# xmed-lab/MOC

Measured on AMD Instinct MI355X. Metric: meta-steps/sec (train), slides/sec (eval) on 16-shot NSCLC synthetic bags, higher is better.
Workload: dtype f32; 1 GPU; NSCLC 2-way 16-shot train loop: 32 slides/epoch x 15000 patches x 512, topj 400, topk 10, row mask on; bag_storage=fp32, arithmetic=fp32 accumulate (MFMA), parallelism=single GPU, one Adam step per slide

## Files before the change

### moc_amd/csrc/moc_meta.hip

```cpp
#include <cstdlib>
#include <cstring>
#include <new>
#include "moc_meta_internal.h"
#include <type_traits>
#include "moc_p2p.h"

int moc_check_batch(const moc_batch_t* B, const char* who);
int moc_launch_topk_mean(const float* keys, int64_t key_stride, const float* vals, int64_t val_stride,
                         const int64_t* seg_off, const int32_t* seg_len, int seg0, int n_seg, int C, int K,
                         int smallest, float* pooled, int32_t* idx_out, int32_t* cnt_out, hipStream_t s);

using namespace moc_meta_internal;

namespace {

struct AdamCoef {
    float wd, one_minus_b1, beta2, one_minus_b2, eps;
    float neg_step_size;
    float bc2_sqrt;
    float grad_scale;
};

__device__ __forceinline__ void adam_update(float& p, float& m, float& v, float g, const AdamCoef& k) {
    g = moc_fadd(g, moc_fmul(k.wd, p));
// ... 634 lines not shown
        for (int sw = 0; sw < 2; ++sw) {
            const int d = dl + sw * dcols;
            if (d < D) {
                float g0 = 0.f, g1 = 0.f;
                for (int p = 0; p < P; ++p) {
                    const float xv = xs[(size_t)p * D + d];
                    g0 = fmaf(dhs[p * H + ha], xv, g0);
                    if (JN > 1) g1 = fmaf(dhs[p * H + ha + 1], xv, g1);
                }
                gr[sw][0] = g0; gr[sw][1] = g1;
            }
        }
    }
    float gt = 0.f;
    int tail = -1;
    if (wg == 0) {
        if (t < 4 * H) {
            const int i = t >> 6, h = t & 63;
            for (int p = 0; p < P; ++p) gt = fmaf(dz[p * 4 + i], H1s[p * H + h], gt);
            tail = H + t;
        } else if (t < 4 * H + 4) {
            const int i = t - 4 * H;
            for (int p = 0; p < P; ++p) gt += dz[p * 4 + i];
            tail = H + 4 * H + i;
        } else if (t >= 320 && t < 320 + H) {
            const int h = t - 320;
            for (int p = 0; p < P; ++p) gt += dhs[p * H + h];
            tail = h;
        }
    }
    if (!a.apply_adam) {
        if (own)
            for (int sw = 0; sw < 2; ++sw) {
                const int d = dl + sw * dcols;
                if (d < D) { g.g_W1[(ha + 0) * D + d] = gr[sw][0]; if (JN > 1) g.g_W1[(ha + 1) * D + d] = gr[sw][1]; }
            }
        if (tail >= H + 4 * H) a.g_b2[tail - 5 * H] = gt;
        else if (tail >= H) a.g_W2[tail - H] = gt;
        else if (tail >= 0) a.g_b1[tail] = gt;
        return;
    }
    if (g.x.world > 1) {
        __shared__ int p2p_ok;
        const int64_t nW1 = (int64_t)H * D;
        if (own)
#pragma unroll
            for (int sw = 0; sw < 2; ++sw) {
                const int d = dl + sw * dcols;
                if (d < D) { p2p_push(g.x, (int64_t)(ha + 0) * D + d, gr[sw][0]); if (JN > 1) p2p_push(g.x, (int64_t)(ha + 1) * D + d, gr[sw][1]); }
            }
        if (tail >= 0) p2p_push(g.x, nW1 + tail, gt);
        if (!p2p_signal_wait(g.x, wg, &p2p_ok)) return;
        if (own)
#pragma unroll
            for (int sw = 0; sw < 2; ++sw) {
                const int d = dl + sw * dcols;
                if (d < D) {
                    gr[sw][0] = p2p_sum(g.x, (int64_t)(ha + 0) * D + d, gr[sw][0]);
                    if (JN > 1) gr[sw][1] = p2p_sum(g.x, (int64_t)(ha + 1) * D + d, gr[sw][1]);
                }
            }
        if (tail >= 0) gt = p2p_sum(g.x, nW1 + tail, gt);
    }
    const float gs = ak.grad_scale;
    if (own) {
#pragma unroll
        for (int sw = 0; sw < 2; ++sw) {
            const int d = dl + sw * dcols;
            if (d < D) {
#pragma unroll
                for (int j = 0; j < 2; ++j) {
                    if (j >= JN) continue;
                    const int e = (ha + j) * D + d;
                    adam_update(pw[j][sw], pm[j][sw], pv[j][sw], gr[sw][j] * gs, ak);
                    g.W1[e] = pw[j][sw]; g.m_W1[e] = pm[j][sw]; g.v_W1[e] = pv[j][sw];
                    w1_image_store(g.img_dt, g.W1img, D, ha + j, d, pw[j][sw]);
                }
            }
        }
    }
    if (tail >= 0) {
        adam_update(pW, pM, pV, gt * gs, ak);
        if (tail >= H + 4 * H) { const int i = tail - 5 * H; a.b2[i] = pW; a.m_b2[i] = pM; a.v_b2[i] = pV; }
        else if (tail >= H) { const int i = tail - H; g.W2out[i] = pW; a.m_W2[i] = pM; a.v_W2[i] = pV; }
        else { a.b1[tail] = pW; a.m_b1[tail] = pM; a.v_b1[tail] = pV; }
    }
    MOC_STAMP(18);
}

struct TileStepArgs {
    const unsigned long long* tkey;
    const uint32_t* trho;
    int64_t slot0;
    int cap, ntile_bound, C, K, D, slide0;
    int n_runs, slide_stride;
    const int32_t* n_sel;
    const int64_t* labels;
    int PS_CAP, xdt;
    int tail_inside;
    int S_host;
    float *W1, *m_W1, *v_W1;
    const float* W2;
    float *b1, *m_b1, *v_b1, *b2, *m_b2, *v_b2, *m_W2, *v_W2;
    int64_t base;
    AdamCoef adam;
    const AdamCoef* adam_tab;
    const int32_t* adam_ctr;
    int adam_pos, apply_adam;
    uint32_t use_bits;
    int img_dt;
    const int64_t* trid;
    const float4* tlam;
    const float4* tsc;
    const float* H1;
    const unsigned char* X;
    float* pooled_out;
    int32_t* topk_idx_out;
    int32_t* topk_cnt_out;
    float* loss;
    int32_t* pred;
    int32_t* n_pair;
    unsigned char* W1img;
    float* W2out;
    float *g_W1, *g_b1, *g_W2, *g_b2;
    const float* mixed_in;
    const float* cand;
    const float* gates;
    const int64_t* sel_row;
    int64_t stride;
    int64_t par_stride, w2_stride, w2out_stride, img_stride;
    const int64_t* row_off;
    int prefetch_next;
    int sink_off;
};
struct TileStepArgsRuns {
    TileStepArgs s;
    int64_t base_r[MOC_MAX_RUNS], slot0_r[MOC_MAX_RUNS];
    int32_t cap_r[MOC_MAX_RUNS], ntb_r[MOC_MAX_RUNS];
};
static_assert(sizeof(TileStepArgsRuns) <= 1024, "a kernel-argument segment over 1 KiB takes a slow launch path (profiles/NOTES.md)");
constexpr int MOC_HP_RUNS = 8;
struct TileStepArgsRunsHp {
    TileStepArgs s;
    int64_t base_r[MOC_HP_RUNS], slot0_r[MOC_HP_RUNS];
    int32_t cap_r[MOC_HP_RUNS], ntb_r[MOC_HP_RUNS];
    AdamCoef adam_r[MOC_HP_RUNS];
};
static_assert(sizeof(TileStepArgsRunsHp) <= 1024, "a kernel-argument segment over 1 KiB takes a slow launch path (profiles/NOTES.md)");
static_assert(offsetof(TileStepArgsRunsHp, adam_r) % sizeof(AdamCoef) == 0, "a run's coefficients: one aligned 32-byte scalar load");
__host__ __device__ __forceinline__ const TileStepArgs& tile_common(const TileStepArgs& x) { return x; }
__host__ __device__ __forceinline__ const TileStepArgs& tile_common(const TileStepArgsRuns& x) { return x.s; }
__host__ __device__ __forceinline__ const TileStepArgs& tile_common(const TileStepArgsRunsHp& x) { return x.s; }

template <int VQ, typename ArgsT>
__global__ __launch_bounds__(256, 4) void pool_w1_step_tiles_kernel(ArgsT args) {
    extern __shared__ __attribute__((aligned(16))) unsigned char smem[];
    constexpr bool RUNS = !std::is_same<ArgsT, TileStepArgs>::value;
    constexpr bool RUN_HP = std::is_same<ArgsT, TileStepArgsRunsHp>::value;
    const TileStepArgs& a = tile_common(args);
    static_assert(offsetof(TileStepArgs, n_sel) + 8 <= 64, "the first loads' arguments must share the first cache line");
    int b = a.slide0;
    int64_t base = 0, slot0 = a.slot0, po = 0, w2o = 0, w2outo = 0, imgo = 0;
    int cap = a.cap, ntile_bound = a.ntile_bound;
    constexpr bool runs = RUNS;
    if constexpr (RUNS) {
        const int run = blockIdx.z;
        b += run * a.slide_stride;
        slot0 = kernarg_at<int64_t>(offsetof(ArgsT, slot0_r) + 8 * (size_t)run);
        cap = kernarg_at<int32_t>(offsetof(ArgsT, cap_r) + 4 * (size_t)run);
        ntile_bound = kernarg_at<int32_t>(offsetof(ArgsT, ntb_r) + 4 * (size_t)run);
    }
    const int C = a.C, K = a.K, D = a.D;
    const int t = threadIdx.x, lane = t & 63, wave = __builtin_amdgcn_readfirstlane(t >> 6);
    const int cb = blockIdx.x, h = blockIdx.y;
    const bool tail_wg = !a.tail_inside && cb == (D >> 8);
    const bool tail_role = a.tail_inside ? cb == 0 : tail_wg;
    const bool wg0 = cb == 0 && h == 0;
    constexpr int CL = 64;
    MOC_STAMP(10);
    MOC_STAMP_MIN(33);
    MOC_STAMP_MAX(34);
    unsigned long long key[VQ];
    uint32_t rho[VQ / 4];
#define MOC_TILE_KEYS(c)                                                                                              \
    {                                                                                                                 \
        const int64_t s_c_ = slot0 + (int64_t)(c) * cap * TILE_R;                                                     \
        const int nrec_b_ = ntile_bound * TILE_R;                                                                     \
        _Pragma("unroll") for (int q = 0; q < VQ; ++q) {                                                              \
            const int j = q * 64 + lane;                                                                              \
            key[q] = a.tkey[s_c_ + (j < nrec_b_ ? j : nrec_b_ - 1)];                                                  \
        }                                                                                                             \
        _Pragma("unroll") for (int rq = 0; rq < VQ / 4; ++rq) {                                                       \
            const int x = rq * 64 + lane;                                                                             \
            rho[rq] = a.trho[slot0 / TILE_R + (int64_t)(c) * cap + (x < ntile_bound ? x : ntile_bound - 1)];          \
        }                                                                                                             \
    }
    if (wave < C) MOC_TILE_KEYS(wave)
    __builtin_amdgcn_sched_barrier(0);
    moc_kernarg_touch<sizeof(ArgsT)>();
    const int PS_CAP = a.PS_CAP;
    base = a.base;
    if constexpr (RUNS) {
        const int run = blockIdx.z;
        base = kernarg_at<int64_t>(offsetof(ArgsT, base_r) + 8 * (size_t)run);
        po = (int64_t)run * a.par_stride; w2o = (int64_t)run * a.w2_stride; w2outo = (int64_t)run * a.w2out_stride;
        imgo = (int64_t)run * a.img_stride;
    }
    const int d = cb * 256 + t;
    float pw = 0.f, pm = 0.f, pv = 0.f;
    float pT = 0.f, pTm = 0.f, pTv = 0.f;
    int tail = -1;
    if (tail_role) {
        if (t < 4) tail = H + t * H + h;
        else if (t == 64) tail = h;
        else if (h == 0 && t >= 128 && t < 132) tail = H + 4 * H + (t - 128);
    }
    float w2v = 0.f;
    if (t < 4) w2v = a.W2[w2o + t * H + h];
    if (a.apply_adam) {
        if (!tail_wg) {
            const int64_t e = po + h * D + d;
            pw = a.W1[e]; pm = a.m_W1[e]; pv = a.v_W1[e];
        }
        if (tail >= H + 4 * H) { const int64_t i = po + tail - 5 * H; pT = a.b2[i]; pTm = a.m_b2[i]; pTv = a.v_b2[i]; }
        else if (tail >= H) { const int64_t i = po + tail - H; pTm = a.m_W2[i]; pTv = a.v_W2[i]; }
        else if (tail >= 0) { pT = a.b1[po + tail]; pTm = a.m_b1[po + tail]; pTv = a.v_b1[po + tail]; }
    }
    MOC_STAMP(19);
    if (wave >= C && a.prefetch_next) {
        const int64_t nb = a.row_off[b + 1];
        const int S2 = a.n_sel[b + 1];
        const int esz_p = a.xdt == MOC_F32 ? 4 : 2;
        const int lpr = D * esz_p / 128;
        const int iw = 4 - C;
        const int gx = (D >> 8) + (a.tail_inside ? 0 : 1);
        const int g0 = ((h * gx + cb) * iw + (wave - C)) * 64 + lane, G = gx * H * iw * 64;
        typedef const __attribute__((address_space(1))) void* gptr_t;
        typedef __attribute__((address_space(3))) void* lptr_t;
        float* sinkw = reinterpret_cast<float*>(smem + a.sink_off) + (wave - C) * 64;
        for (int L = g0; L < S2 * lpr; L += G) {
            const int r = L / lpr;
            const unsigned char* pl = a.X + a.sel_row[nb + r] * (int64_t)D * esz_p + (int64_t)(L - r * lpr) * 128;
            __builtin_amdgcn_global_load_lds((gptr_t)pl, (lptr_t)sinkw, 4, 0, 0);
        }
        const int ncol = 2 * C + 2, lpc = (S2 + 31) >> 5;
        for (int L = g0; L < ncol * lpc; L += G) {
            const int c = L / lpc;
            const float* pl = a.cand + (int64_t)c * a.stride + nb + (int64_t)(L - c * lpc) * 32;
            __builtin_amdgcn_global_load_lds((gptr_t)pl, (lptr_t)sinkw, 4, 0, 0);
        }
    }
    AdamCoef ak = a.adam;
    if (a.adam_tab) ak = a.adam_tab[a.adam_ctr[0] + a.adam_pos];
    if constexpr (RUN_HP) ak = kernarg_at<AdamCoef>(offsetof(ArgsT, adam_r) + sizeof(AdamCoef) * (size_t)blockIdx.z);
    const int S = (!RUNS && a.S_host >= 0) ? a.S_host : a.n_sel[b];
    const int y = (int)a.labels[b];
    const int k = K < S ? K : S;
    float4* plam = reinterpret_cast<float4*>(smem);
    float4* psc = plam + (size_t)C * K;
    float* xs = reinterpret_cast<float*>(psc + (size_t)C * K);
    float* dhs = xs + (size_t)C * K * 256;
    float* dz = dhs + (((size_t)C * K + 3) & ~(size_t)3);
    unsigned long long* list = reinterpret_cast<unsigned long long*>(dz + (size_t)C * K * 4);
    unsigned long long* t0s = list + (size_t)C * PS_CAP;
    int64_t* prid = reinterpret_cast<int64_t*>(t0s + C);
    int* lsrc = reinterpret_cast<int*>(prid + (size_t)C * K);
    float* topv = reinterpret_cast<float*>(lsrc + (size_t)C * CL);
    float* pooled_s = topv + (size_t)C * 16;
    float* dpool = pooled_s + C;
    int* ncand = reinterpret_cast<int*>(dpool + C);
    int* flagc = ncand + C;
    int* topk_s = flagc + C;
    float* h1s = reinterpret_cast<float*>(topk_s + C * K);
    float* w2s = h1s + (size_t)C * K;
    if (t < 4) { w2s[t] = w2v; if (tail >= H) pT = w2v; }
    const int ntile = (S + 15) >> 4;
    for (int c = wave; c < C; c += 4) {
        const int64_t s_c = slot0 + (int64_t)c * cap * TILE_R;
        if (c != wave) MOC_TILE_KEYS(c)
        if (lane == 0) ncand[c] = 0;
        uint32_t hi[VQ];
        uint32_t m = 0u;
        const int nrec = ntile * TILE_R;
#pragma unroll
        for (int q = 0; q < VQ; ++q) {
            hi[q] = q * 64 + lane < nrec ? (uint32_t)(key[q] >> 32) : 0u;
            m = hi[q] > m ? hi[q] : m;
        }
        MOC_STAMP(20);
        {
            const uint32_t o1 = (uint32_t)__builtin_amdgcn_update_dpp(0, (int)m, 0xB1, 0xf, 0xf, false);
            m = o1 > m ? o1 : m;
            const uint32_t o2 = (uint32_t)__builtin_amdgcn_update_dpp(0, (int)m, 0x4E, 0xf, 0xf, false);
            m = o2 > m ? o2 : m;
        }
        const uint32_t gm = (uint32_t)__shfl((int)m, (lane & 15) * 4, 64);
        int grank = 0;
#define MOC_ROR(n) grank += (uint32_t)__builtin_amdgcn_update_dpp(0, (int)gm, 0x120 + n, 0xf, 0xf, false) > gm ? 1 : 0;
        MOC_ROR(1) MOC_ROR(2) MOC_ROR(3) MOC_ROR(4) MOC_ROR(5) MOC_ROR(6) MOC_ROR(7) MOC_ROR(8)
        MOC_ROR(9) MOC_ROR(10) MOC_ROR(11) MOC_ROR(12) MOC_ROR(13) MOC_ROR(14) MOC_ROR(15)
#undef MOC_ROR
        const unsigned long long hit = __ballot(lane < 16 && grank == k - 1 && gm != 0u);
        uint32_t T0 = 0u;
        if (hit != 0ull) T0 = (uint32_t)__builtin_amdgcn_readlane((int)gm, __ffsll((long long)hit) - 1);
        const uint32_t T1 = T0 > 1u ? T0 : 1u;
        int cnt = 0;
#pragma unroll
        for (int q = 0; q < VQ; ++q)
            if (q * 64 < nrec) cnt += hi[q] >= T1 ? 1 : 0;
        if (cnt > 0) {
            int pos = atomicAdd(&ncand[c], cnt);
#pragma unroll
            for (int q = 0; q < VQ; ++q) {
                if (q * 64 < nrec && hi[q] >= T1) {
                    if (pos < CL) {
                        list[(size_t)c * PS_CAP + pos] = key[q];
                        lsrc[c * CL + pos] = q * 64 + lane;
                    }
                    ++pos;
                }
            }
        }
        bool bad = false;
#pragma unroll
        for (int rq = 0; rq < VQ / 4; ++rq)
            bad = bad || (rq * 64 + lane < ntile && rho[rq] != 0u && rho[rq] >= T0);
        asm volatile("s_waitcnt lgkmcnt(0)" ::: "memory");
        __builtin_amdgcn_wave_barrier();
        const int n = ncand[c];
        const bool fall = __ballot(bad) != 0ull || n > CL || n < k || k <= 0;
        if (lane == 0) { flagc[c] = fall ? 1 : 0; t0s[c] = (unsigned long long)T0 << 32; }
        MOC_STAMP(11);
        if (!fall) {
            const unsigned long long mine = lane < n ? list[(size_t)c * PS_CAP + lane] : 0ull;
            const int jrec = lane < n ? lsrc[c * CL + lane] : 0;
            const int64_t rid = a.trid[s_c + jrec];
            const float4 lam = a.tlam[s_c + jrec];
            const float4 scv = a.tsc[s_c + jrec];
            int rank = 0;
            for (int l = 0; l < n; ++l) rank += list[(size_t)c * PS_CAP + l] > mine ? 1 : 0;
            MOC_STAMP(12);
            if (lane < n && rank < k) {
                topk_s[c * K + rank] = (int)(~(unsigned)mine);
                topv[c * 16 + rank] = key_to_float((unsigned)(mine >> 32));
                const int p = c * k + rank;
                prid[p] = rid; plam[p] = lam; psc[p] = scv;
            }
            asm volatile("s_waitcnt lgkmcnt(0)" ::: "memory");
            __builtin_amdgcn_wave_barrier();
            if (lane == 0) {
                float sum = 0.f;
                for (int r = 0; r < k; ++r) sum += topv[c * 16 + r];
                pooled_s[c] = sum / (float)k;
                if (wg0) {
                    a.pooled_out[(int64_t)b * C + c] = pooled_s[c];
                    if (a.topk_cnt_out) a.topk_cnt_out[(int64_t)b * C + c] = k;
                }
            }
            if (a.topk_idx_out && wg0)
                for (int r = lane; r < K; r += 64)
                    a.topk_idx_out[((int64_t)b * C + c) * K + r] = r < k ? topk_s[c * K + r] : -1;
        }
    }
    __syncthreads();
    MOC_STAMP(13);
    bool fast = true;
    for (int c = 0; c < C; ++c) fast = fast && flagc[c] == 0;
    if (wg0 && t == 0 && a.n_pair) {
        if (a.n_runs > 0) atomicMax(a.n_pair, fast ? MOC_TILE_PATH_RECORDS : MOC_TILE_PATH_FULL);
        else *a.n_pair = fast ? MOC_TILE_PATH_RECORDS : MOC_TILE_PATH_FULL;
    }
    if (!fast) {
        if (t < C) ncand[t] = 0;
        __syncthreads();
        for (int c = 0; c < C; ++c) {
            const unsigned long long T0 = t0s[c];
            const float* col = a.mixed_in + (int64_t)c * a.stride + base;
            for (int i = t; i < S; i += 256) {
                const unsigned long long kk = ((unsigned long long)moc_key_desc(col[i]) << 32) | (unsigned)(~(unsigned)i);
                if (kk >= T0) {
                    const int pos = atomicAdd(&ncand[c], 1);
                    if (pos < PS_CAP) list[(size_t)c * PS_CAP + pos] = kk;
                }
            }
        }
        __syncthreads();
        for (int c = wave; c < C; c += 4) {
            const int n = ncand[c];
            const bool overflow = n > PS_CAP;
            const float* col = a.mixed_in + (int64_t)c * a.stride + base;
            unsigned long long prev = ~0ull;
            float sum = 0.f;
            for (int r = 0; r < k; ++r) {
                unsigned long long best = 0ull;
                if (!overflow) {
                    for (int i = lane; i < n; i += 64) {
                        const unsigned long long v = list[(size_t)c * PS_CAP + i];
                        if (v < prev && v > best) best = v;
                    }
                } else {
                    for (int i = lane; i < S; i += 64) {
                        const unsigned long long v = ps_key(col, i, S);
                        if (v < prev && v > best) best = v;
                    }
                }
                best = wave_max_u64(best);
                prev = best;
                sum += key_to_float((unsigned)(best >> 32));
                if (lane == 0) topk_s[c * K + r] = (int)(~(unsigned)best);
            }
            if (lane == 0) pooled_s[c] = k > 0 ? sum / (float)k : __uint_as_float(0x7FC00000u);
            __builtin_amdgcn_wave_barrier();
            if (lane == 0 && wg0) {
                a.pooled_out[(int64_t)b * C + c] = pooled_s[c];
                if (a.topk_cnt_out) a.topk_cnt_out[(int64_t)b * C + c] = k;
            }
            if (a.topk_idx_out && wg0)
                for (int r = lane; r < K; r += 64)
                    a.topk_idx_out[((int64_t)b * C + c) * K + r] = r < k ? topk_s[c * K + r] : -1;
        }
        __syncthreads();
        const int P0 = C * k;
        for (int p = t; p < P0; p += 256) {
            const unsigned kinv0 = (65536u + (unsigned)k - 1u) / (unsigned)k;
            const int c = (int)(((unsigned)p * kinv0) >> 16);
            const int sidx = topk_s[c * K + (p - c * k)];
            prid[p] = a.sel_row[base + sidx];
            plam[p] = reinterpret_cast<const float4*>(a.gates)[base + sidx];
            float4 s4;
            s4.x = a.cand[(int64_t)c * a.stride + base + sidx];
            s4.y = a.cand[(int64_t)(C + c) * a.stride + base + sidx];
            s4.z = a.cand[(int64_t)(2 * C) * a.stride + base + sidx];
            s4.w = a.cand[(int64_t)(2 * C + 1) * a.stride + base + sidx];
            psc[p] = s4;
        }
        __syncthreads();
    }
    MOC_STAMP(14);
    MOC_STAMP(15);
    const int P = C * k;
    if (P > 0) {
        const unsigned kinv = (65536u + (unsigned)k - 1u) / (unsigned)k;
        if (wave == 3) {
            for (int p = lane; p < P; p += 64) {
                const int c = (int)(((unsigned)p * kinv) >> 16);
                h1s[p] = a.H1[(base + topk_s[c * K + (p - c * k)]) * H + h];
            }
        } else if (!tail_wg) {
            const int esz = a.xdt == MOC_F32 ? 4 : 2;
            const int64_t col0 = (int64_t)cb * 256 * esz;
            constexpr int RF = 8;
            for (int p0 = wave; p0 < P; p0 += 3 * RF) {
                const unsigned char* rp[RF];
#pragma unroll
                for (int u = 0; u < RF; ++u) {
                    const int pu = p0 + 3 * u;
                    rp[u] = a.X + prid[pu < P ? pu : p0] * (int64_t)D * esz + col0;
                }
                float4 v[RF];
                if (a.xdt == MOC_F32) {
#pragma unroll
                    for (int u = 0; u < RF; ++u) v[u] = reinterpret_cast<const float4*>(rp[u])[lane];
                } else {
                    const bool f16 = a.xdt == MOC_F16;
                    auto widen = [&](uint2 raw) {
                        float4 o;
                        if (f16) {
                            o.x = moc_f16_to_f32((uint16_t)raw.x); o.y = moc_f16_to_f32((uint16_t)(raw.x >> 16));
                            o.z = moc_f16_to_f32((uint16_t)raw.y); o.w = moc_f16_to_f32((uint16_t)(raw.y >> 16));
                        } else {
                            o.x = __uint_as_float(raw.x << 16); o.y = __uint_as_float(raw.x & 0xFFFF0000u);
                            o.z = __uint_as_float(raw.y << 16); o.w = __uint_as_float(raw.y & 0xFFFF0000u);
                        }
                        return o;
                    };
                    uint2 raw[RF];
#pragma unroll
                    for (int u = 0; u < RF; ++u) raw[u] = reinterpret_cast<const uint2*>(rp[u])[lane];
#pragma unroll
                    for (int u = 0; u < RF; ++u) v[u] = widen(raw[u]);
                }
#pragma unroll
                for (int u = 0; u < RF; ++u) {
                    const int pu = p0 + 3 * u;
                    if (pu < P) reinterpret_cast<float4*>(xs + (size_t)pu * 256)[lane] = v[u];
                }
            }
        }
    }
    if (wave == 3) {
        const float xv = lane < C ? pooled_s[lane] : -INFINITY;
        float mx = xv;
        int arg = lane < C ? lane : 0x7fffffff;
        for (int off = 8; off > 0; off >>= 1) {
            const float om = __shfl_xor(mx, off, 64);
            const int oa = __shfl_xor(arg, off, 64);
            if (om > mx || (om == mx && oa < arg)) { mx = om; arg = oa; }
        }
        const float ex = lane < C ? expf(xv - mx) : 0.f;
        float se = ex;
        for (int off = 8; off > 0; off >>= 1) se += __shfl_xor(se, off, 64);
        const float lse = mx + logf(se);
        if (lane < C) dpool[lane] = expf(xv - lse) - (lane == y ? 1.f : 0.f);
        if (lane == 0 && wg0) {
            a.loss[b] = lse - pooled_s[y];
            a.pred[b] = arg;
        }
    }
    __syncthreads();
    MOC_STAMP(16);
    for (int p = t; p < P; p += 256) {
        const unsigned kinv = (65536u + (unsigned)k - 1u) / (unsigned)k;
        const int c = (int)(((unsigned)p * kinv) >> 16);
        const float gk = dpool[c] / (float)k;
        const float4 l4 = plam[p], s4 = psc[p];
        const float lamv[4] = {l4.x, l4.y, l4.z, l4.w}, scs[4] = {s4.x, s4.y, s4.z, s4.w};
        float v = 0.f;
#pragma unroll
        for (int i = 0; i < 4; ++i) {
            const float dlam = (a.use_bits >> i & 1u) ? gk * scs[i] : 0.f;
            const float dzi = dlam * lamv[i] * (1.f - lamv[i]);
            dz[p * 4 + i] = dzi;
            v = fmaf(dzi, w2s[i], v);
        }
        dhs[p] = h1s[p] > 0.f ? v : 0.f;
    }
    __syncthreads();
    MOC_STAMP(17);
    float gr = 0.f;
    if (!tail_wg) {
        int p = 0;
        for (; p + 4 <= P; p += 4) {
            const float4 d4 = *reinterpret_cast<const float4*>(dhs + p);
            const float x0 = xs[(size_t)p * 256 + t], x1 = xs[(size_t)(p + 1) * 256 + t];
            const float x2 = xs[(size_t)(p + 2) * 256 + t], x3 = xs[(size_t)(p + 3) * 256 + t];
            gr = fmaf(d4.x, x0, gr); gr = fmaf(d4.y, x1, gr); gr = fmaf(d4.z, x2, gr); gr = fmaf(d4.w, x3, gr);
        }
        for (; p < P; ++p) gr = fmaf(dhs[p], xs[(size_t)p * 256 + t], gr);
    }
    float gt = 0.f;
    if (tail >= H + 4 * H) {
        const int i = tail - 5 * H;
        int p = 0;
        for (; p + 4 <= P; p += 4) {
            const float z0 = dz[p * 4 + i], z1 = dz[(p + 1) * 4 + i], z2 = dz[(p + 2) * 4 + i], z3 = dz[(p + 3) * 4 + i];
            gt += z0; gt += z1; gt += z2; gt += z3;
        }
        for (; p < P; ++p) gt += dz[p * 4 + i];
    } else if (tail >= H) {
        int p = 0;
        for (; p + 4 <= P; p += 4) {
            const float z0 = dz[p * 4 + t], z1 = dz[(p + 1) * 4 + t], z2 = dz[(p + 2) * 4 + t], z3 = dz[(p + 3) * 4 + t];
            const float4 h4 = {h1s[p], h1s[p + 1], h1s[p + 2], h1s[p + 3]};
            gt = fmaf(z0, h4.x, gt); gt = fmaf(z1, h4.y, gt); gt = fmaf(z2, h4.z, gt); gt = fmaf(z3, h4.w, gt);
        }
        for (; p < P; ++p) gt = fmaf(dz[p * 4 + t], h1s[p], gt);
    } else if (tail >= 0) {
        int p = 0;
        for (; p + 4 <= P; p += 4) {
            const float4 d4 = *reinterpret_cast<const float4*>(dhs + p);
            gt += d4.x; gt += d4.y; gt += d4.z; gt += d4.w;
        }
        for (; p < P; ++p) gt += dhs[p];
    }
    if (!a.apply_adam) {
        if (!tail_wg) a.g_W1[h * D + d] = gr;
        if (tail >= H + 4 * H) a.g_b2[tail - 5 * H] = gt;
        else if (tail >= H) a.g_W2[tail - H] = gt;
        else if (tail >= 0) a.g_b1[tail] = gt;
        return;
    }
    const float gs = ak.grad_scale;
    if (!tail_wg) {
        const int64_t e = po + h * D + d;
        adam_update(pw, pm, pv, gr * gs, ak);
        a.W1[e] = pw; a.m_W1[e] = pm; a.v_W1[e] = pv;
        w1_image_store(a.img_dt, a.W1img + imgo, D, h, d, pw);
    }
    if (tail >= 0) {
        adam_update(pT, pTm, pTv, gt * gs, ak);
        if (tail >= H + 4 * H) { const int64_t i = po + tail - 5 * H; a.b2[i] = pT; a.m_b2[i] = pTm; a.v_b2[i] = pTv; }
        else if (tail >= H) { const int i = tail - H; a.W2out[w2outo + i] = pT; a.m_W2[po + i] = pTm; a.v_W2[po + i] = pTv; }
        else { a.b1[po + tail] = pT; a.m_b1[po + tail] = pTm; a.v_b1[po + tail] = pTv; }
    }
    MOC_STAMP(18);
    MOC_STAMP_MAX(35);
}
#undef MOC_TILE_KEYS

constexpr int WD_PCH_MIN = 128;


__global__ __launch_bounds__(1024) void pool_w1_step_wide_kernel(FusedArgs g, float* pooled_out, int32_t* topk_idx_out,
                                                                 int32_t* topk_cnt_out, int PS_CAP, int region_bytes,
                                                                 int external_pool, int WD_PCH) {
    extern __shared__ __attribute__((aligned(16))) unsigned char smem[];
    const FinishArgs& a = g.f;
    const int b = a.slide0, C = a.C, K = a.K, D = a.D;
    const int wg = blockIdx.x, t = threadIdx.x, lane = t & 63, wave = t >> 6;
    const int DS = D / 16, d_lo = wg * DS;
    moc_kernarg_touch<sizeof(FusedArgs)>();
    MOC_STAMP(40);
    const int esz = a.xdt == MOC_F32 ? 4 : 2;
    const int PMAX = C * K;
    unsigned char* region = smem;
    unsigned long long* list = reinterpret_cast<unsigned long long*>(region);
    unsigned long long* wmax = reinterpret_cast<unsigned long long*>(smem + region_bytes);
    float* pooled_s = reinterpret_cast<float*>(wmax + (size_t)C * 16);
    float* dpool = pooled_s + C;
    int* ncand = reinterpret_cast<int*>(dpool + C);
    int* topk_s = ncand + C;
    float* dz = reinterpret_cast<float*>(smem + (((reinterpret_cast<unsigned char*>(topk_s + PMAX) - smem) + 15) & ~(ptrdiff_t)15));
    float* h1o = dz + (size_t)(PMAX + 16) * 4;
    const int PM = (PMAX + 16 + 3) & ~3;
    unsigned* mask = reinterpret_cast<unsigned*>(h1o + (size_t)PMAX * 4);
    int* sidx_s = reinterpret_cast<int*>(mask + (size_t)PM * 2);
    float* W2s = reinterpret_cast<float*>(sidx_s + PMAX);
    float* red = W2s + 4 * H;
    int64_t* prow_s = reinterpret_cast<int64_t*>(smem + (((reinterpret_cast<unsigned char*>(red + 32) - smem) + 7) & ~(ptrdiff_t)7));

    const int NTN = DS / 16;
    const bool has_tile = wave < 4 * NTN;
    const bool ksplit = 4 * NTN <= 8;
    const int twave = ksplit ? (wave & 7) : wave;
    const bool in_product = ksplit || has_tile;
    const int h0 = (twave / NTN) * 16, d0 = d_lo + (twave % NTN) * 16;
    float pw[4], pm[4], pv[4];
#pragma unroll
    for (int i = 0; i < 4; ++i) {
        pw[i] = pm[i] = pv[i] = 0.f;
        if (has_tile && a.apply_adam) {
            const int e = (h0 + (lane >> 4) * 4 + i) * D + d0 + (lane & 15);
            pw[i] = g.W1[e]; pm[i] = g.m_W1[e]; pv[i] = g.v_W1[e];
        }
    }
    const AdamCoef ak = step_coef(a);
    const float w2r = t < 4 * H ? a.W2[t] : 0.f;
    float pS = 0.f, pSm = 0.f, pSv = 0.f;
    int small = -1;
    if (t < 16) small = H + (t >> 2) * H + wg * 4 + (t & 3);
    else if (t < 20) small = wg * 4 + (t - 16);
    else if (t < 24 && wg == 0) small = H + 4 * H + (t - 20);
    if (small >= 0 && a.apply_adam) {
        if (small >= 5 * H) { pS = a.b2[small - 5 * H]; pSm = a.m_b2[small - 5 * H]; pSv = a.v_b2[small - 5 * H]; }
        else if (small >= H) { pS = a.W2[small - H]; pSm = a.m_W2[small - H]; pSv = a.v_W2[small - H]; }
        else { pS = a.b1[small]; pSm = a.m_b1[small]; pSv = a.v_b1[small]; }
    }
    int64_t base;
    int k, P;
    unsigned kinv;
    float4 hv_pre[5];
    auto request_hidden = [&]() {
#pragma unroll
        for (int q = 0; q < 5; ++q) {
            const int e = t + q * 1024;
            hv_pre[q] = float4{0.f, 0.f, 0.f, 0.f};
            if (e < P * 16) {
                const int p = e >> 4, c = (int)(((unsigned)p * kinv) >> 16);
                hv_pre[q] = *reinterpret_cast<const float4*>(a.H1 + (base + topk_s[c * K + (p - c * k)]) * H + (e & 15) * 4);
            }
        }
    };
    auto zero_masks = [&]() {
        for (int p = t; p < 2 * P; p += 1024) mask[(p >= P ? PM - P : 0) + p] = 0u;
        if (t < 64) dz[P * 4 + t] = 0.f;
    };
    if (external_pool) {
        base = a.base_host >= 0 ? a.base_host : a.row_off[b];
        const int y = (int)a.labels[b];
        const int PK = C * K;
        const int own_idx = a.topk_idx[(int64_t)b * PK + (t < PK ? t : PK - 1)];
        k = a.topk_cnt[(int64_t)b * C];
        const float pooled_v = a.pooled[(int64_t)b * C + (t < C ? t : 0)];
        P = C * k;
        kinv = k > 0 ? (65536u + (unsigned)k - 1u) / (unsigned)k : 0u;
        const unsigned kinvK = (65536u + (unsigned)K - 1u) / (unsigned)K;
        const int own_c = (int)(((unsigned)t * kinvK) >> 16), own_pos = t - own_c * K;
        const bool own = t < PK && own_pos < k;
        int64_t own_row = 0;
        float sc[4] = {0.f, 0.f, 0.f, 0.f};
// ... 453 lines not shown
}
int wide_pch(const moc_batch_t* B) {
    int pch = (B->C * B->topk + 31) & ~31;
    while (pch > WD_PCH_MIN && wide_smem(B, pch) > (size_t)FS_MAX_DYN_LDS) pch -= 32;
    return pch < WD_PCH_MIN ? WD_PCH_MIN : pch;
}
}

StepPlan moc_meta_internal::step_plan(const moc_batch_t* B, const moc_meta_ws_t* ws, bool exchange, int train) {
    static const bool tiles_off = getenv("MOC_TILE_RECORDS") && atoi(getenv("MOC_TILE_RECORDS")) == 0;
    StepPlan p = {};
    const int sb = s_bound(B);
    p.cap = B->C <= 8 ? PS_CAP_MAX : PS_CAP_MAX / 2;
    p.pool_one = B->topk <= 16 && B->C <= 16 && sb <= 64 * 16 * PS_VPT && (!train || B->C * B->topk <= 64);
    if (!train || !ws->W2_alt) return p;
    const size_t lds = FS_MAX_DYN_LDS, narrow = fused_step_smem(B, p.cap), tiles = tiles_step_smem(B, p.cap);
    if (p.pool_one && B->D <= 1024 && (int64_t)B->C * B->topk * B->D <= FS_MAX_XS && narrow <= lds) {
        p.kind = STEP_NARROW; p.smem = narrow;
        const bool records = ws->tile_ws && B->row_off_host &&
                             ws->tile_ws_bytes >= (int64_t)tile_bytes(tile_slots(B->total_rows, B->n_slides, B->C));
        if (!exchange && !tiles_off && records && moc_cdiv(sb, 16) * TILE_R <= 16 * 64 && tiles <= lds) {
            p.kind = STEP_TILES; p.smem = tiles;
        }
        return p;
    }
    if (B->topk <= 16 && B->C <= 64 && B->D % 512 == 0 && B->D <= 1024 && wide_smem(B, WD_PCH_MIN) <= lds) {
        p.kind = STEP_WIDE; p.pch = wide_pch(B); p.wide_cap = wide_cap(B);
        p.wide_region = (int)wide_region(B, p.pch); p.smem = wide_smem(B, p.pch);
        p.external = sb > 8192 || (int64_t)B->C * sb > 49152;
    }
    return p;
}

namespace {

int step_attrs() {
    static std::once_flag once;
    static char failed[96] = "";
    std::call_once(once, [] {
        auto raise = [](const char* name, const void* f, int bytes) {
            if (!failed[0] && hipFuncSetAttribute(f, hipFuncAttributeMaxDynamicSharedMemorySize, bytes) != hipSuccess)
                snprintf(failed, sizeof(failed), "%s to %d bytes", name, bytes);
        };
        raise("finish_kernel", (const void*)finish_kernel, 159 * 1024);
        raise("pool_step_kernel", (const void*)pool_step_kernel, 160 * 1024);
        raise("pool_w1_step_kernel", (const void*)pool_w1_step_kernel, FS_MAX_DYN_LDS);
        raise("pool_w1_step_wide_kernel", (const void*)pool_w1_step_wide_kernel, FS_MAX_DYN_LDS);
#define MOC_TILES_ATTR(VQ)                                                                                                    \
        raise("pool_w1_step_tiles_kernel", (const void*)pool_w1_step_tiles_kernel<VQ, TileStepArgs>, FS_MAX_DYN_LDS);        \
        raise("pool_w1_step_tiles_kernel(runs)", (const void*)pool_w1_step_tiles_kernel<VQ, TileStepArgsRuns>, FS_MAX_DYN_LDS); \
        raise("pool_w1_step_tiles_kernel(runs_hp)", (const void*)pool_w1_step_tiles_kernel<VQ, TileStepArgsRunsHp>, FS_MAX_DYN_LDS)
        MOC_TILES_ATTR(4); MOC_TILES_ATTR(8); MOC_TILES_ATTR(12); MOC_TILES_ATTR(16);
#undef MOC_TILES_ATTR
    });
    if (failed[0]) MOC_FAIL(MOC_ELAUNCH, "moc_fused_step: cannot raise the dynamic LDS limit of %s", failed);
    return MOC_OK;
}

FinishArgs finish_args(const moc_batch_t* B, const moc_meta_t* M, const moc_meta_ws_t* ws, const int64_t* labels, int slide0,
                       int train, int apply_adam, uint32_t use_bits, const AdamCoef& k) {
    FinishArgs a = {};
    a.row_off = B->row_off; a.sel_row = B->sel_row; a.n_sel = B->n_sel; a.cand = B->cand;
    a.H1 = ws->H1; a.gates = ws->gates; a.pooled = ws->pooled;
    a.labels = labels; a.loss = ws->loss; a.pred = ws->pred;
    a.W2 = M->W2; a.b2 = M->b2; a.b1 = M->b1;
    a.m_W2 = M->m_W2; a.m_b2 = M->m_b2; a.m_b1 = M->m_b1; a.v_W2 = M->v_W2; a.v_b2 = M->v_b2; a.v_b1 = M->v_b1;
    a.g_W2 = M->g_W2; a.g_b2 = M->g_b2; a.g_b1 = M->g_b1;
    a.stride = B->total_rows; a.C = B->C; a.K = B->topk; a.slide0 = slide0; a.train = train;
    a.apply_adam = apply_adam; a.use_bits = use_bits; a.adam = k;
    return a;
}
void finish_rows(FinishArgs& a, const moc_batch_t* B, const moc_meta_ws_t* ws, int slide, bool one_slide) {
    a.mixed_in = ws->mixed;
    a.X = (const unsigned char*)B->X; a.D = B->D; a.xdt = B->dtype;
    a.base_host = -1; a.seg_host = 0;
    if (one_slide && B->row_off_host) {
        a.base_host = B->row_off_host[slide];
        a.seg_host = (int)(B->row_off_host[slide + 1] - a.base_host);
    }
}

int launch_finish(const moc_batch_t* B, const moc_meta_t* M, const moc_meta_ws_t* ws, const int64_t* labels,
                  int slide0, int n, int train, int apply_adam, uint32_t use_bits, const AdamCoef& k, hipStream_t s) {
    FinishArgs a = finish_args(B, M, ws, labels, slide0, train, apply_adam, use_bits, k);
    a.topk_idx = ws->topk_idx; a.topk_cnt = ws->topk_cnt;
    a.pair_dh = ws->pair_dh; a.pair_row = ws->pair_row; a.n_pair = ws->n_pair;
    const size_t smem = train ? (size_t)B->C * B->topk * (4 * sizeof(float) + sizeof(int)) +
                                (size_t)(FIN_CHUNK + 4) * H * sizeof(float) : 0;
    MOC_REQUIRE(smem <= 159 * 1024, "finish: C*topk = %d too large", B->C * B->topk);
    finish_kernel<<<n, 256, smem, s>>>(a);
    MOC_CHECK_LAUNCH("moc_finish");
    return MOC_OK;
}

int launch_pool_finish(const StepPlan& p, const moc_batch_t* B, const moc_meta_t* M, const moc_meta_ws_t* ws, const int64_t* labels,
                       int slide0, int n, int train, int apply_adam, uint32_t use_bits, const AdamCoef& k, hipStream_t s) {
    if (!p.pool_one) {
        if (int rc = launch_pool(B, ws, slide0, n, s)) return rc;
        return launch_finish(B, M, ws, labels, slide0, n, train, apply_adam, use_bits, k, s);
    }
    FinishArgs a = finish_args(B, M, ws, labels, slide0, train, apply_adam, use_bits, k);
    finish_rows(a, B, ws, slide0, n == 1);
    a.pair_dh = ws->pair_dh; a.pair_row = ws->pair_row; a.n_pair = ws->n_pair;
    const size_t C = B->C, K = B->topk, PK = train ? C * K : 0;
    const size_t smem = C * p.cap * 8 + C * 16 * 8 + C * 4 * 3 + C * K * 4 + PK * (4 * 4 + 2 * H * 4) + 4 * H * 4;
    pool_step_kernel<<<n, 1024, smem, s>>>(a, ws->pooled, ws->topk_idx, ws->topk_cnt, p.cap);
    MOC_CHECK_LAUNCH("moc_pool_step");
    return MOC_OK;
}

struct StepTab { const AdamCoef* tab; const int32_t* ctr; int pos; };

void tile_region(const moc_batch_t* B, int slide, int64_t* slot0, int* tcap, int* tb) {
    const int64_t base = B->row_off_host[slide], seg = B->row_off_host[slide + 1] - base;
    *tcap = moc_cdiv(seg, 16) > 0 ? moc_cdiv(seg, 16) : 1;
    int tb_all = moc_cdiv(s_bound(B), 16);
    if (B->n_sel_host) {
        const int sh = B->n_sel_host[slide];
        if (sh >= 0 && moc_cdiv(sh, 16) < tb_all) tb_all = sh > 0 ? moc_cdiv(sh, 16) : 1;
    }
    *tb = *tcap < tb_all ? *tcap : tb_all;
    *slot0 = ((base >> 4) + slide) * (int64_t)B->C * TILE_R;
}

TileStepArgs tile_step_args(const StepPlan& p, const moc_batch_t* B, const moc_meta_t* M, const moc_meta_ws_t* ws, const int64_t* labels, int slide,
                            uint32_t use_bits, const AdamCoef& k, float* W2out, int apply_adam, const StepTab* tab) {
    const TileWs T = tile_carve(ws->tile_ws, tile_slots(B->total_rows, B->n_slides, B->C));
    TileStepArgs ta = {};
    ta.tkey = T.key; ta.trho = T.rho; ta.trid = T.rid; ta.tlam = T.lam; ta.tsc = T.sc;
    tile_region(B, slide, &ta.slot0, &ta.cap, &ta.ntile_bound);
    ta.C = B->C; ta.K = B->topk; ta.D = B->D; ta.slide0 = slide; ta.PS_CAP = p.cap;
    ta.xdt = B->dtype; ta.n_sel = B->n_sel; ta.labels = labels;
    ta.W1 = M->W1; ta.m_W1 = M->m_W1; ta.v_W1 = M->v_W1; ta.W2 = M->W2;
    ta.b1 = M->b1; ta.m_b1 = M->m_b1; ta.v_b1 = M->v_b1; ta.b2 = M->b2; ta.m_b2 = M->m_b2; ta.v_b2 = M->v_b2;
    ta.m_W2 = M->m_W2; ta.v_W2 = M->v_W2;
    ta.base = B->row_off_host[slide]; ta.adam = k;
    ta.row_off = B->row_off; ta.prefetch_next = 0;
    ta.S_host = B->n_sel_host ? B->n_sel_host[slide] : -1;
    ta.sink_off = (int)(p.smem - TILES_SINK);
    if (tab) { ta.adam_tab = tab->tab; ta.adam_ctr = tab->ctr; ta.adam_pos = tab->pos; }
    ta.apply_adam = apply_adam; ta.use_bits = use_bits; ta.img_dt = B->dtype;
    ta.H1 = ws->H1; ta.X = (const unsigned char*)B->X;
    ta.pooled_out = ws->pooled; ta.topk_idx_out = ws->topk_idx; ta.topk_cnt_out = ws->topk_cnt;
    ta.loss = ws->loss; ta.pred = ws->pred; ta.n_pair = ws->n_pair;
    ta.W1img = (unsigned char*)M->W1_image; ta.W2out = W2out;
    ta.g_W1 = M->g_W1; ta.g_b1 = M->g_b1; ta.g_W2 = M->g_W2; ta.g_b2 = M->g_b2;
    ta.mixed_in = ws->mixed; ta.cand = B->cand; ta.gates = ws->gates; ta.sel_row = B->sel_row; ta.stride = B->total_rows;
    return ta;
}

template <typename ArgsT>
int launch_tile_step_as(const StepPlan& p, const moc_batch_t* B, const ArgsT& args, int runs, int tb, hipStream_t s) {
    const TileStepArgs& ta = tile_common(args);
    const dim3 grid(B->D / 256 + (ta.tail_inside ? 0 : 1), H, runs);
#define MOC_TILES_LAUNCH(VQ) pool_w1_step_tiles_kernel<VQ, ArgsT><<<grid, 256, p.smem, s>>>(args)
    const int vq = moc_cdiv((int64_t)tb * TILE_R, 64);
    if (vq <= 4) MOC_TILES_LAUNCH(4);
    else if (vq <= 8) MOC_TILES_LAUNCH(8);
    else if (vq <= 12) MOC_TILES_LAUNCH(12);
    else MOC_TILES_LAUNCH(16);
#undef MOC_TILES_LAUNCH
    MOC_CHECK_LAUNCH("moc_fused_step(tiles)");
    return MOC_OK;
}
template <typename RunsT>
int launch_tile_step_runs(const StepPlan& p, const moc_batch_t* B, const RunsT& tr, hipStream_t s) {
    int tb = tr.s.ntile_bound;
    for (int r = 0; r < tr.s.n_runs; ++r) tb = tr.ntb_r[r] > tb ? tr.ntb_r[r] : tb;
    return launch_tile_step_as(p, B, tr, tr.s.n_runs, tb, s);
}

bool step_prefetch_on() {
    static const bool on = !(getenv("MOC_STEP_PREFETCH") && atoi(getenv("MOC_STEP_PREFETCH")) == 0);
    return on;
}
int launch_fused_step(const StepPlan& p, const moc_batch_t* B, const moc_meta_t* M, const moc_meta_ws_t* ws, const int64_t* labels,
                      int slide, uint32_t use_bits, const AdamCoef& k, float* W2out, hipStream_t s,
                      int apply_adam = 1, const P2pArgs* x = nullptr, const StepTab* tab = nullptr, int next_slide = -1) {
    MOC_REQUIRE(p.one_launch() && !(p.tiles() && x), "moc_fused_step: plan of kind %d%s", (int)p.kind, x ? " with a gradient exchange" : "");
    if (p.tiles()) {
        TileStepArgs ta = tile_step_args(p, B, M, ws, labels, slide, use_bits, k, W2out, apply_adam, tab);
        if (step_prefetch_on() && next_slide == slide + 1 && next_slide < B->n_slides && B->C < 4) ta.prefetch_next = 1;
        return launch_tile_step_as(p, B, ta, 1, ta.ntile_bound, s);
    }
    FusedArgs g = {};
    if (x) g.x = *x;
    g.f = finish_args(B, M, ws, labels, slide, 1, apply_adam, use_bits, k);
    FinishArgs& a = g.f;
    finish_rows(a, B, ws, slide, true);
    if (tab) { a.adam_tab = tab->tab; a.adam_ctr = tab->ctr; a.adam_pos = tab->pos; }
    g.g_W1 = M->g_W1; g.W1 = M->W1; g.m_W1 = M->m_W1; g.v_W1 = M->v_W1; g.W1img = (unsigned char*)M->W1_image;
    g.W2out = W2out; g.img_dt = B->dtype;
    if (p.kind == STEP_WIDE) {
        if (p.external) {
            if (int rc = launch_pool(B, ws, slide, 1, s)) return rc;
            a.topk_idx = ws->topk_idx; a.topk_cnt = ws->topk_cnt;
        }
        pool_w1_step_wide_kernel<<<H / 4, 1024, p.smem, s>>>(g, ws->pooled, ws->topk_idx, ws->topk_cnt, p.wide_cap, p.wide_region,
                                                             p.external, p.pch);
        MOC_CHECK_LAUNCH("moc_fused_step(wide)");
        return MOC_OK;
    }
    pool_w1_step_kernel<<<g.x.world > 1 ? H / 4 : H / 2, 1024, p.smem, s>>>(g, ws->pooled, ws->topk_idx, ws->topk_cnt, p.cap);
    MOC_CHECK_LAUNCH("moc_fused_step");
    return MOC_OK;
}

int launch_w1(const moc_batch_t* B, const moc_meta_t* M, const moc_meta_ws_t* ws, int apply_adam,
              const AdamCoef& k, hipStream_t s, bool padded_pairs) {
    W1Args a;
    a.P_static = padded_pairs ? B->C * B->topk : -1;
    a.W1img = (unsigned char*)M->W1_image;
    a.X = (const unsigned char*)B->X; a.pair_dh = ws->pair_dh; a.pair_row = ws->pair_row; a.n_pair = ws->n_pair;
    a.W1 = M->W1; a.m_W1 = M->m_W1; a.v_W1 = M->v_W1; a.g_W1 = M->g_W1; a.D = B->D; a.apply_adam = apply_adam; a.adam = k;
    const dim3 grid(B->D / 256, H / 8);
    if (B->dtype == MOC_F16) w1_update_kernel<true, true><<<grid, 256, 0, s>>>(a);
    else if (B->dtype == MOC_BF16) w1_update_kernel<true><<<grid, 256, 0, s>>>(a);
    else w1_update_kernel<false><<<grid, 256, 0, s>>>(a);
    MOC_CHECK_LAUNCH("moc_w1_update");
    return MOC_OK;
}

}

extern "C" int moc_pool_loss(const moc_batch_t* B, const moc_meta_ws_t* ws, const int64_t* labels,
                             int slide0, int n, moc_stream_t stream) {
    if (int rc = moc_check_batch(B, "moc_pool_loss")) return rc;
    MOC_REQUIRE(ws && labels, "moc_pool_loss: null ws/labels");
    MOC_REQUIRE(slide0 >= 0 && n >= 1 && slide0 + n <= B->n_slides, "moc_pool_loss: bad slide range");
    MOC_REQUIRE(B->C <= 256, "moc_pool_loss: C > 256");
    hipStream_t s = (hipStream_t)stream;
    (void)step_attrs();
    moc_meta_t none = {};
    AdamCoef k = {};
    return launch_pool_finish(step_plan(B, ws, false, 0), B, &none, ws, labels, slide0, n, 0, 0, 0, k, s);
}

extern "C" int moc_ce_loss(const float* pooled, const int64_t* labels, int n, int C, float* loss, int32_t* pred,
                           moc_stream_t stream) {
    MOC_REQUIRE(pooled && labels && loss && pred, "moc_ce_loss: null pointer");
    MOC_REQUIRE(n >= 1 && C >= 1 && C <= 256, "moc_ce_loss: bad n=%d C=%d (C <= 256)", n, C);
    FinishArgs a = {};
    a.pooled = pooled; a.labels = labels; a.loss = loss; a.pred = pred; a.C = C; a.slide0 = 0; a.train = 0;
    finish_kernel<<<n, 256, 0, (hipStream_t)stream>>>(a);
    MOC_CHECK_LAUNCH("moc_ce_loss");
    return MOC_OK;
}

extern "C" int moc_train_grad(const moc_batch_t* B, const moc_meta_t* M, const moc_meta_ws_t* ws,
                              const int64_t* labels, int slide, uint32_t use_bits, moc_stream_t stream) {
    if (int rc = moc_check_batch(B, "moc_train_grad")) return rc;
    if (int rc = check_meta(B, M, ws, "moc_train_grad", false, true)) return rc;
    MOC_REQUIRE(labels && slide >= 0 && slide < B->n_slides, "moc_train_grad: bad labels/slide");
    hipStream_t s = (hipStream_t)stream;
    if (int rc = step_attrs()) return rc;
    const StepPlan p = step_plan(B, ws, false);
    AdamCoef k = {};
    k.grad_scale = 1.f;
    if (int rc = launch_w1_images(B, M, nullptr, s)) return rc;
    if (int rc = launch_forward(B, M, ws, slide, 1, use_bits, s, p.tiles())) return rc;
    if (p.one_launch()) return launch_fused_step(p, B, M, ws, labels, slide, use_bits, k, nullptr, s, 0);
    if (int rc = launch_pool_finish(p, B, M, ws, labels, slide, 1, 1, 0, use_bits, k, s)) return rc;
    return launch_w1(B, M, ws, 0, k, s, p.pool_one);
}

extern "C" int moc_senet_backward(const void* X, int dtype, int64_t S, int D, const float* H1, const float* gates,
                                  const float* grad_gates, const float* W2, float* g_W1, float* g_b1, float* g_W2, float* g_b2,
                                  float* pair_dz, float* pair_dh, int64_t* pair_row, int32_t* n_pair, moc_stream_t stream) {
    MOC_REQUIRE(X && H1 && gates && grad_gates && W2 && g_W1 && g_b1 && g_W2 && g_b2 && pair_dz && pair_dh && pair_row && n_pair,
                "moc_senet_backward: null pointer");
    MOC_REQUIRE(dtype == MOC_F32 || dtype == MOC_BF16 || dtype == MOC_F16, "moc_senet_backward: bad dtype %d", dtype);
    MOC_REQUIRE(S >= 1 && D > 0 && D % 256 == 0, "moc_senet_backward: bad shape S=%lld D=%d (D a multiple of 256)", (long long)S, D);
    hipStream_t s = (hipStream_t)stream;
    senet_bwd_rows_kernel<<<1, 1024, 0, s>>>(H1, gates, grad_gates, W2, S, pair_dz, pair_dh, pair_row, n_pair, g_b1, g_W2, g_b2);
    MOC_CHECK_LAUNCH("moc_senet_backward(rows)");
    W1Args a = {};
    a.P_static = -1;
    a.X = (const unsigned char*)X; a.pair_dh = pair_dh; a.pair_row = pair_row; a.n_pair = n_pair;
    a.g_W1 = g_W1; a.D = D; a.apply_adam = 0;
    const dim3 grid(D / 256, H / 8);
    if (dtype == MOC_F16) w1_update_kernel<true, true><<<grid, 256, 0, s>>>(a);
    else if (dtype == MOC_BF16) w1_update_kernel<true><<<grid, 256, 0, s>>>(a);
    else w1_update_kernel<false><<<grid, 256, 0, s>>>(a);
    MOC_CHECK_LAUNCH("moc_senet_backward(W1)");
    return MOC_OK;
}

extern "C" int moc_adam_step(const moc_meta_t* M, float grad_scale, moc_stream_t stream) {
    MOC_REQUIRE(M && M->H == H && M->D > 0, "moc_adam_step: bad meta");
    MOC_REQUIRE(M->W1 && M->m_W1 && M->v_W1 && M->g_W1 && M->b1 && M->m_b1 && M->v_b1 && M->g_b1 &&
                M->W2 && M->m_W2 && M->v_W2 && M->g_W2 && M->b2 && M->m_b2 && M->v_b2 && M->g_b2,
                "moc_adam_step: null tensor");
    const AdamCoef k = adam_coef(M, M->step + 1, grad_scale);
    const int n = H * M->D + H + 4 * H + 4;
    adam_all_kernel<<<moc_cdiv(n, 256), 256, 0, (hipStream_t)stream>>>(*M, M->D, k, nullptr, 0);
    MOC_CHECK_LAUNCH("moc_adam_step");
    return MOC_OK;
}

extern "C" int moc_train_steps_dp(const moc_batch_t* B, const moc_meta_t* M, const moc_meta_ws_t* ws,
                                  const int64_t* labels, int slide0, int n, uint32_t use_bits,
                                  float* grad_flat, int64_t grad_count, moc_allreduce_fn allreduce,
                                  void* comm, int world, moc_stream_t stream) {
    if (int rc = moc_check_batch(B, "moc_train_steps_dp")) return rc;
    if (int rc = check_meta(B, M, ws, "moc_train_steps_dp", true, true)) return rc;
    MOC_REQUIRE(labels && slide0 >= 0 && n >= 1 && slide0 + n <= B->n_slides, "moc_train_steps_dp: bad labels/slide range");
// ... 495 lines not shown
```

Before: 52450 meta-steps/s.

## Replace LDS atomics and block barrier with wave-local ballot compaction and DPP reductions

Candidate compaction now uses per-wave ballot plus mbcnt prefix counts instead of an LDS atomicAdd and a reload of the count. The top-k sum uses readlane instead of serial LDS reads, and the softmax reductions use row-of-sixteen DPP swizzles instead of shuffles. The per-pair gradient loop is folded into wave 3 with the H1 gather, which removes one __syncthreads. This relies on C*topk fitting in one wave, now enforced by a host check.

```diff
diff --git a/moc_amd/csrc/moc_meta.hip b/moc_amd/csrc/moc_meta.hip
--- a/moc_amd/csrc/moc_meta.hip
+++ b/moc_amd/csrc/moc_meta.hip
@@ -810,6 +810,18 @@
 __host__ __device__ __forceinline__ const TileStepArgs& tile_common(const TileStepArgsRuns& x) { return x.s; }
 __host__ __device__ __forceinline__ const TileStepArgs& tile_common(const TileStepArgsRunsHp& x) { return x.s; }
 
+template <int OFF>
+__device__ __forceinline__ int row16_xor(int x) {
+    static_assert(OFF == 8 || OFF == 4 || OFF == 2 || OFF == 1, "partners within a row of sixteen");
+    if constexpr (OFF == 8) return __builtin_amdgcn_update_dpp(0, x, 0x128, 0xf, 0xf, false);
+    else if constexpr (OFF == 4)
+        return __builtin_amdgcn_update_dpp(0, __builtin_amdgcn_update_dpp(0, x, 0x141, 0xf, 0xf, false), 0x1B, 0xf, 0xf, false);
+    else if constexpr (OFF == 2) return __builtin_amdgcn_update_dpp(0, x, 0x4E, 0xf, 0xf, false);
+    else return __builtin_amdgcn_update_dpp(0, x, 0xB1, 0xf, 0xf, false);
+}
+template <int OFF>
+__device__ __forceinline__ float row16_xor(float x) { return __uint_as_float((unsigned)row16_xor<OFF>((int)__float_as_uint(x))); }
+
 template <int VQ, typename ArgsT>
 __global__ __launch_bounds__(256, 4) void pool_w1_step_tiles_kernel(ArgsT args) {
     extern __shared__ __attribute__((aligned(16))) unsigned char smem[];
@@ -936,7 +948,6 @@
     for (int c = wave; c < C; c += 4) {
         const int64_t s_c = slot0 + (int64_t)c * cap * TILE_R;
         if (c != wave) MOC_TILE_KEYS(c)
-        if (lane == 0) ncand[c] = 0;
         uint32_t hi[VQ];
         uint32_t m = 0u;
         const int nrec = ntile * TILE_R;
@@ -962,30 +973,25 @@
         uint32_t T0 = 0u;
         if (hit != 0ull) T0 = (uint32_t)__builtin_amdgcn_readlane((int)gm, __ffsll((long long)hit) - 1);
         const uint32_t T1 = T0 > 1u ? T0 : 1u;
-        int cnt = 0;
-#pragma unroll
-        for (int q = 0; q < VQ; ++q)
-            if (q * 64 < nrec) cnt += hi[q] >= T1 ? 1 : 0;
-        if (cnt > 0) {
-            int pos = atomicAdd(&ncand[c], cnt);
-#pragma unroll
-            for (int q = 0; q < VQ; ++q) {
-                if (q * 64 < nrec && hi[q] >= T1) {
-                    if (pos < CL) {
-                        list[(size_t)c * PS_CAP + pos] = key[q];
-                        lsrc[c * CL + pos] = q * 64 + lane;
-                    }
-                    ++pos;
+        int n = 0;
+#pragma unroll
+        for (int q = 0; q < VQ; ++q) {
+            if (q * 64 < nrec) {
+                const bool in = (q * 64 + lane < nrec ? (uint32_t)(key[q] >> 32) : 0u) >= T1;
+                const unsigned long long bq = __ballot(in);
+                const int pos = n + (int)__builtin_amdgcn_mbcnt_hi((uint32_t)(bq >> 32), __builtin_amdgcn_mbcnt_lo((uint32_t)bq, 0u));
+                if (in && pos < CL) {
+                    list[(size_t)c * PS_CAP + pos] = key[q];
+                    lsrc[c * CL + pos] = q * 64 + lane;
                 }
+                n += __popcll(bq);
             }
         }
         bool bad = false;
 #pragma unroll
         for (int rq = 0; rq < VQ / 4; ++rq)
             bad = bad || (rq * 64 + lane < ntile && rho[rq] != 0u && rho[rq] >= T0);
-        asm volatile("s_waitcnt lgkmcnt(0)" ::: "memory");
         __builtin_amdgcn_wave_barrier();
-        const int n = ncand[c];
         const bool fall = __ballot(bad) != 0ull || n > CL || n < k || k <= 0;
         if (lane == 0) { flagc[c] = fall ? 1 : 0; t0s[c] = (unsigned long long)T0 << 32; }
         MOC_STAMP(11);
@@ -1004,11 +1010,12 @@
                 const int p = c * k + rank;
                 prid[p] = rid; plam[p] = lam; psc[p] = scv;
             }
-            asm volatile("s_waitcnt lgkmcnt(0)" ::: "memory");
             __builtin_amdgcn_wave_barrier();
+            const float tv = lane < k ? topv[c * 16 + lane] : 0.f;
+            float sum = 0.f;
+#pragma nounroll
+            for (int r = 0; r < k; ++r) sum += __uint_as_float((unsigned)__builtin_amdgcn_readlane((int)__float_as_uint(tv), r));
             if (lane == 0) {
-                float sum = 0.f;
-                for (int r = 0; r < k; ++r) sum += topv[c * 16 + r];
                 pooled_s[c] = sum / (float)k;
                 if (wg0) {
                     a.pooled_out[(int64_t)b * C + c] = pooled_s[c];
@@ -1097,14 +1104,53 @@
     MOC_STAMP(14);
     MOC_STAMP(15);
     const int P = C * k;
-    if (P > 0) {
-        const unsigned kinv = (65536u + (unsigned)k - 1u) / (unsigned)k;
-        if (wave == 3) {
-            for (int p = lane; p < P; p += 64) {
-                const int c = (int)(((unsigned)p * kinv) >> 16);
-                h1s[p] = a.H1[(base + topk_s[c * K + (p - c * k)]) * H + h];
-            }
-        } else if (!tail_wg) {
+    if (wave == 3) {
+        float hv = 0.f;
+        int pc = 0;
+        if (lane < P) {
+            const unsigned kinv = (65536u + (unsigned)k - 1u) / (unsigned)k;
+            pc = (int)(((unsigned)lane * kinv) >> 16);
+            hv = a.H1[(base + topk_s[pc * K + (lane - pc * k)]) * H + h];
+        }
+        const float xv = lane < C ? pooled_s[lane] : -INFINITY;
+        float mx = xv;
+        int arg = lane < C ? lane : 0x7fffffff;
+#define MOC_CE_MAX(OFF)                                                                                               \
+        {                                                                                                             \
+            const float om = row16_xor<OFF>(mx);                                                                      \
+            const int oa = row16_xor<OFF>(arg);                                                                       \
+            if (om > mx || (om == mx && oa < arg)) { mx = om; arg = oa; }                                             \
+        }
+        MOC_CE_MAX(8) MOC_CE_MAX(4) MOC_CE_MAX(2) MOC_CE_MAX(1)
+#undef MOC_CE_MAX
+        const float ex = lane < C ? expf(xv - mx) : 0.f;
+        float se = ex;
+        se += row16_xor<8>(se); se += row16_xor<4>(se); se += row16_xor<2>(se); se += row16_xor<1>(se);
+        const float lse = mx + logf(se);
+        if (lane < C) dpool[lane] = expf(xv - lse) - (lane == y ? 1.f : 0.f);
+        if (lane == 0 && wg0) {
+            a.loss[b] = lse - pooled_s[y];
+            a.pred[b] = arg;
+        }
+        __builtin_amdgcn_wave_barrier();
+        if (lane < P) {
+            const int p = lane;
+            h1s[p] = hv;
+            const float gk = dpool[pc] / (float)k;
+            const float4 l4 = plam[p], s4 = psc[p];
+            const float lamv[4] = {l4.x, l4.y, l4.z, l4.w}, scs[4] = {s4.x, s4.y, s4.z, s4.w};
+            float v = 0.f;
+#pragma unroll
+            for (int i = 0; i < 4; ++i) {
+                const float dlam = (a.use_bits >> i & 1u) ? gk * scs[i] : 0.f;
+                const float dzi = dlam * lamv[i] * (1.f - lamv[i]);
+                dz[p * 4 + i] = dzi;
+                v = fmaf(dzi, w2s[i], v);
+            }
+            dhs[p] = hv > 0.f ? v : 0.f;
+        }
+    } else if (P > 0) {
+        if (!tail_wg) {
             const int esz = a.xdt == MOC_F32 ? 4 : 2;
             const int64_t col0 = (int64_t)cb * 256 * esz;
             constexpr int RF = 8;
@@ -1146,44 +1192,8 @@
             }
         }
     }
-    if (wave == 3) {
-        const float xv = lane < C ? pooled_s[lane] : -INFINITY;
-        float mx = xv;
-        int arg = lane < C ? lane : 0x7fffffff;
-        for (int off = 8; off > 0; off >>= 1) {
-            const float om = __shfl_xor(mx, off, 64);
-            const int oa = __shfl_xor(arg, off, 64);
-            if (om > mx || (om == mx && oa < arg)) { mx = om; arg = oa; }
-        }
-        const float ex = lane < C ? expf(xv - mx) : 0.f;
-        float se = ex;
-        for (int off = 8; off > 0; off >>= 1) se += __shfl_xor(se, off, 64);
-        const float lse = mx + logf(se);
-        if (lane < C) dpool[lane] = expf(xv - lse) - (lane == y ? 1.f : 0.f);
-        if (lane == 0 && wg0) {
-            a.loss[b] = lse - pooled_s[y];
-            a.pred[b] = arg;
-        }
-    }
     __syncthreads();
     MOC_STAMP(16);
-    for (int p = t; p < P; p += 256) {
-        const unsigned kinv = (65536u + (unsigned)k - 1u) / (unsigned)k;
-        const int c = (int)(((unsigned)p * kinv) >> 16);
-        const float gk = dpool[c] / (float)k;
-        const float4 l4 = plam[p], s4 = psc[p];
-        const float lamv[4] = {l4.x, l4.y, l4.z, l4.w}, scs[4] = {s4.x, s4.y, s4.z, s4.w};
-        float v = 0.f;
-#pragma unroll
-        for (int i = 0; i < 4; ++i) {
-            const float dlam = (a.use_bits >> i & 1u) ? gk * scs[i] : 0.f;
-            const float dzi = dlam * lamv[i] * (1.f - lamv[i]);
-            dz[p * 4 + i] = dzi;
-            v = fmaf(dzi, w2s[i], v);
-        }
-        dhs[p] = h1s[p] > 0.f ? v : 0.f;
-    }
-    __syncthreads();
     MOC_STAMP(17);
     float gr = 0.f;
     if (!tail_wg) {
@@ -1943,6 +1953,7 @@
 template <typename ArgsT>
 int launch_tile_step_as(const StepPlan& p, const moc_batch_t* B, const ArgsT& args, int runs, int tb, hipStream_t s) {
     const TileStepArgs& ta = tile_common(args);
+    MOC_REQUIRE(B->C * B->topk <= 64, "moc_fused_step(tiles): C * topk = %d pairs, one wave forms at most 64", B->C * B->topk);
     const dim3 grid(B->D / 256 + (ta.tail_inside ? 0 : 1), H, runs);
 #define MOC_TILES_LAUNCH(VQ) pool_w1_step_tiles_kernel<VQ, ArgsT><<<grid, 256, p.smem, s>>>(args)
     const int vq = moc_cdiv((int64_t)tb * TILE_R, 64);
```

Result: faster. 55290 meta-steps/s (median of 6 runs) (+5.4%).
